# morispi/CONSENT

Measured on AMD Instinct MI355X. Metric: corrected windows/sec, higher is better.
Workload: dtype u8/int16 (2-bit bases, integer DP); 1 GPU; pacbio_d150_msa150: synthetic PacBio-profile piles, 500 bp windows, depth 150, maxMSA 150, k=9, solid=4, commonKMers=8, minAnchors=2; distinct_windows_per_run=704512, engines_per_gpu=4, engines_requested=4, engine_allocation_runs=0, hw_queues=4, overflow_windows=0, template_fallback_windows=0

## Files before the change

consent_amd/csrc/cw_index.h:

```cpp
#ifndef CW_INDEX_H
#define CW_INDEX_H

#include "cw_device.h"

typedef __attribute__((address_space(3))) uint32_t* cw_l32w;
typedef __attribute__((address_space(3))) const uint32_t* cw_l32;
typedef __attribute__((address_space(1))) const uint32_t* cw_g32;
typedef __attribute__((address_space(3))) uint16_t* cw_l16w;
typedef __attribute__((address_space(1))) uint16_t* cw_g16w;
#define CW_IDX_THREADS 1024
#define CW_IDX_WAVES 16
#define CW_IDX_LDS_BYTES 163840
#define CW_TMAX 2048
#define CW_EX_SLOTS 1024
#define CW_EX_BITS 10
#define CW_EXP_SLOTS 8
#define CW_EXG_SLOTS 262144
#define CW_TH_SLOTS 4096
#ifndef CW_IDX_BYTES_MIN_N
#define CW_IDX_BYTES_MIN_N 64u
#endif
#define CW_IDX_STAGE_OFF 139776
#define CW_IDX_STAGE_N 192
#define CW_IDX_STAGE_WORDS ((CW_IDX_LDS_BYTES - CW_IDX_STAGE_OFF - 16 - CW_IDX_STAGE_N * 8) / 4)

enum CwIdxRoute : unsigned {
    CW_IR_STAGED = 1u << 0,
    CW_IR_BYTES_DONE = 1u << 1,
    CW_IR_NIBBLES = 1u << 2,
    CW_IR_BIG_EX = 1u << 3,
    CW_IR_EXPORT_MASKS = 1u << 4,
    CW_IR_EXPORT_WALK = 1u << 5,
    CW_IR_REWALK = 1u << 6,
    CW_IR_HASHED = 1u << 7,
    CW_IR_HASH_PASSES = 1u << 8,
    CW_IR_HASH_GSORT = 1u << 9,
    CW_IR_WIDE = 1u << 10,
    CW_IR_TFIT = 1u << 11,
    CW_IR_PG = 1u << 12,
    CW_IR_HIT_LIST = 1u << 13,
    CW_IR_USE_BITS = 1u << 14
};
#ifdef CW_TEST_AIDS
#define CW_IDX_ROUTE(ctr, cond, bits) do { if (cond) atomicOr(&(ctr)->prof[CW_PS_IDX_ROUTE], (unsigned long long)(bits)); } while (0)
#else
#define CW_IDX_ROUTE(ctr, cond, bits) do { } while (0)
#endif

__host__ __device__ __forceinline__ uint32_t cw_ab_np(uint32_t N) { uint32_t Np = (N + 1u) & ~1u; if (((Np >> 1) & 1u) == 0u) Np += 2u; return Np; }
__host__ __device__ __forceinline__ uint64_t cw_ab_align(uint64_t x) { return (x + 15ull) & ~15ull; }
#define CW_AB_HDR 64u
#define CW_AB_ROWS_MAX 254u
__host__ __device__ __forceinline__ uint32_t cw_ab_ap(uint32_t A) { return (A + 15u) & ~15u; }
template <typename B> struct CwAbCarve {
    B hdr;
    B ckey;
    B pres;
    B dirty;
    B badm;
    B rowid;
    B delta;
    B P;
    B end;
};
template <typename B> __host__ __device__ __forceinline__ CwAbCarve<B> cw_ab_carve(B blk, uint32_t A, uint32_t N, uint32_t n_dirty, uint32_t n_rows) {
    const uint32_t Np = cw_ab_np(N), Nw = (N + 63u) >> 6;
    CwAbCarve<B> c;
    c.hdr = blk;
    c.ckey = blk + CW_AB_HDR;
    c.pres = c.ckey + cw_ab_align((uint64_t)A * 4);
    c.dirty = c.pres + cw_ab_align((uint64_t)A * Nw * 8);
    c.badm = c.dirty + cw_ab_align((uint64_t)n_dirty * 2);
    c.rowid = c.badm + cw_ab_align((uint64_t)A * 8);
    c.delta = c.rowid + cw_ab_align((uint64_t)A);
// ... 105 lines not shown
__device__ __forceinline__ int cw_tpl_lookup(const uint32_t* th, const uint32_t* tkey, uint32_t key) {
    uint32_t bkt = CW_TH_HOME(key);
    const uint32_t fp = CW_TH_FP(key);
    for (;;) {
        for (uint32_t j = 0; j < 4u; ++j) {
            const uint32_t e = th[bkt * 4u + j];
            if (e == 0) return -1;
            if ((e & ~4095u) == fp && tkey[CW_TH_POS(e) - 1] == key) return (int)CW_TH_POS(e) - 1;
        }
        bkt = (bkt + 1) & (CW_TH_BUCKETS - 1);
    }
}

#define CW_IDX_EX_OFF 131072u
#define CW_IDX_SCAN_OFF (CW_IDX_EX_OFF + CW_EX_SLOTS * 8u)
static_assert(CW_IDX_SCAN_OFF + 512u == CW_IDX_STAGE_OFF, "the staged pile starts behind the 512 B of flags and scan scratch");
template <uint32_t T> struct IdxTplOff {
    static constexpr uint32_t tkey = CW_TH_SLOTS * 4u, tsup = tkey + 4u * T, trep = tsup + 4u * T, tcand = trep + T, cand_tp = tcand + 2u * T,
                              seen = cand_tp + 2u * T, misc = seen + CW_IDX_WAVES * (T / 32u) * 4u, P = misc + 256u;
};
static_assert(IdxTplOff<1024>::tsup == 20480u && IdxTplOff<1024>::trep == 24576u && IdxTplOff<1024>::tcand == 25600u && IdxTplOff<1024>::cand_tp == 27648u &&
              IdxTplOff<1024>::seen == 29696u && IdxTplOff<1024>::misc == 31744u && IdxTplOff<1024>::P == 32000u, "the narrow layout");
static_assert(IdxTplOff<2048>::tsup == 24576u && IdxTplOff<2048>::trep == 32768u && IdxTplOff<2048>::tcand == 34816u && IdxTplOff<2048>::cand_tp == 38912u &&
              IdxTplOff<2048>::seen == 43008u && IdxTplOff<2048>::misc == 47104u && IdxTplOff<2048>::P == 47360u, "the wide layout");
static_assert(IdxTplOff<2048>::P < CW_IDX_STAGE_OFF && IdxTplOff<CW_TMAX>::P == IdxTplOff<2048>::P, "the position matrix stops short of the staged pile");

struct IdxLds {
    uint8_t* lds;
    bool wide;
    __device__ __forceinline__ uint32_t* tab() const { return (uint32_t*)lds; }
    __device__ __forceinline__ unsigned long long* ex() const { return (unsigned long long*)(lds + CW_IDX_EX_OFF); }
    __device__ __forceinline__ uint32_t* scan_tmp() const { return (uint32_t*)(lds + CW_IDX_SCAN_OFF); }
    __device__ __forceinline__ uint32_t* flags() const { return scan_tmp() + 32; }
    __device__ __forceinline__ uint32_t* st_hdr() const { return (uint32_t*)(lds + CW_IDX_STAGE_OFF); }
    __device__ __forceinline__ uint32_t* s_len() const { return st_hdr() + 4; }
    __device__ __forceinline__ uint32_t* s_off() const { return s_len() + CW_IDX_STAGE_N; }
    __device__ __forceinline__ uint32_t* s_words() const { return s_off() + CW_IDX_STAGE_N; }
    typedef IdxTplOff<1024> O1; typedef IdxTplOff<2048> O2;
    __device__ __forceinline__ uint32_t* th() const { return (uint32_t*)lds; }
    __device__ __forceinline__ uint32_t* tkey() const { return (uint32_t*)(lds + O1::tkey); }
    __device__ __forceinline__ uint32_t* tsup() const { return (uint32_t*)(lds + (wide ? O2::tsup : O1::tsup)); }
    __device__ __forceinline__ uint8_t* trep() const { return lds + (wide ? O2::trep : O1::trep); }
    __device__ __forceinline__ int16_t* tcand() const { return (int16_t*)(lds + (wide ? O2::tcand : O1::tcand)); }
    __device__ __forceinline__ uint16_t* cand_tp() const { return (uint16_t*)(lds + (wide ? O2::cand_tp : O1::cand_tp)); }
    __device__ __forceinline__ uint32_t* seen() const { return (uint32_t*)(lds + (wide ? O2::seen : O1::seen)); }
    __device__ __forceinline__ uint32_t seen_words() const { return wide ? 64u : 32u; }
    __device__ __forceinline__ uint32_t* misc() const { return (uint32_t*)(lds + (wide ? O2::misc : O1::misc)); }
    __device__ __forceinline__ uint16_t* P() const { return (uint16_t*)(lds + (wide ? O2::P : O1::P)); }
    __device__ __forceinline__ uint32_t p_cap() const { return (CW_IDX_STAGE_OFF - (wide ? O2::P : O1::P)) / 2u; }
};

struct IdxWin {
    WinInfo* wi;
    uint32_t N, L0, solid_base, solid_cap, ab_cap, ab_base, n_kmers;
    __device__ __forceinline__ explicit IdxWin(WinInfo* w) : wi(w), N(w->n_seqs), L0(w->tpl_len), solid_base(w->solid_base), solid_cap(w->solid_cap),
                                                             ab_cap(w->ab_cap), ab_base(w->ab_base), n_kmers(w->n_kmers) {}
};

struct IdxPile {
    uint32_t N, s0;
    bool stm, stw;
    const uint32_t* s_len; const uint32_t* s_off; const uint32_t* s_words;
    const uint32_t* seq_len; const uint64_t* seq_word_off; const uint32_t* bases;
};

struct IdxMatrix {
    uint16_t* P_lds; uint16_t* P_glb;
    const uint16_t* cand_tp;
    bool pg;
    bool tfit;
    uint32_t Np;
    __device__ __forceinline__ uint32_t rd(const uint32_t i) const { return pg ? (uint32_t)((cw_g16w)P_glb)[i] : (uint32_t)((cw_l16w)P_lds)[i]; }
    __device__ __forceinline__ void wr(const uint32_t i, const uint32_t v) const { if (pg) ((cw_g16w)P_glb)[i] = (uint16_t)v; else ((cw_l16w)P_lds)[i] = (uint16_t)v; }
    __device__ __forceinline__ uint32_t row(const uint32_t a) const { return tfit ? (uint32_t)cand_tp[a] : a; }
    __device__ __forceinline__ void clear_lds(const uint32_t n16) const {
        const uint32_t nv = n16 >> 3, pat = (uint32_t)CW_NONE16 * 0x00010001u;
        for (uint32_t i = threadIdx.x; i < nv; i += CW_IDX_THREADS) ((uint4*)P_lds)[i] = make_uint4(pat, pat, pat, pat);
        for (uint32_t i = (nv << 3) + threadIdx.x; i < n16; i += CW_IDX_THREADS) P_lds[i] = (uint16_t)CW_NONE16;
    }
};
__device__ __forceinline__ uint64_t idx_matrix_need(const uint32_t rows, const uint32_t N, const uint32_t Np) {
    return (uint64_t)rows * Np * 2 + (uint64_t)rows * ((N + 63u) >> 6) * 8 + (uint64_t)N * 2 + 16;
}

__device__ __forceinline__ unsigned long long* idx_wg_scratch(const DevScratch& sc) { return sc.ex_fallback + (size_t)blockIdx.x * CW_EXG_SLOTS; }

__device__ __forceinline__ void idx_stop(WinInfo* wi, BatchCounters* ctr, const uint32_t why) { wi->status = CW_WIN_OVERFLOW; wi->pad_ = why; ctr->any_overflow = 1; }

enum IdxShape { IDX_8x128, IDX_8x128_ROT, IDX_2x512, IDX_WAVE };

template <typename W> __device__ __forceinline__ uint64_t idx_window(const W words, const uint32_t p, const uint32_t nwd) {
    const uint32_t wi_ = p >> 4;
    const uint64_t x_ = ((uint64_t)words[wi_] << 32) | (wi_ + 1u < nwd ? words[wi_ + 1u] : 0u);
    return x_ << (2u * (p & 15u));
}
__device__ __forceinline__ uint32_t idx_key_top(const uint64_t x, const uint32_t k) { return (uint32_t)(x >> (64u - 2u * k)); }
__device__ __forceinline__ uint32_t idx_key_field(const uint32_t yh, const uint32_t q, const uint32_t k) { return yh >> (32u - 2u * k - 2u * q); }
__device__ __forceinline__ void idx_keys4(uint64_t x_, const uint32_t k, const uint32_t kmask, uint32_t (&key4)[4]) {
    if (k <= 13u) {
        const uint32_t yh = (uint32_t)(x_ >> 32);
#pragma unroll
        for (uint32_t q = 0; q < 4u; ++q) key4[q] = idx_key_field(yh, q, k) & kmask;
    } else {
// ... 180 lines not shown
}
template <uint32_t KPW, typename Accept, typename CountOf>
__device__ __forceinline__ bool idx_export_masks(const uint32_t (&m)[8], const uint32_t* tab, const uint32_t NI, const uint32_t key_base, const uint32_t out_base,
                                                 uint32_t* scan_tmp, uint32_t* solid_key, uint32_t* solid_cnt, uint32_t& total, Accept&& accept, CountOf&& count_of) {
    const uint32_t lane = threadIdx.x & 63u;
    const uint32_t qbase = (threadIdx.x >> 6) * (NI * 64u) + lane;
    uint32_t offs[8], wtot = 0;
#pragma unroll
    for (int i = 0; i < 8; ++i) {
        const uint32_t c = (uint32_t)__popc(m[i]);
        const uint32_t inc = (uint32_t)cw_wave_scan_add((int)c);
        offs[i] = wtot + inc - c;
        wtot += (uint32_t)cw_lane_value((int)inc, 63);
    }
    uint32_t woff = cw_block_exscan(lane == 0 ? wtot : 0u, scan_tmp, &total);
    woff = (uint32_t)cw_lane_value((int)woff, 0);
    if (!accept(total)) return false;
#pragma unroll
    for (int i = 0; i < 8; ++i) {
        uint32_t mm = m[i], o = out_base + woff + offs[i];
        const uint32_t wd0 = (qbase + (uint32_t)i * 64u) * 4u;
        while (mm) {
            const uint32_t bpos = (uint32_t)__ffs((int)mm) - 1u;
            mm &= mm - 1u;
            const uint32_t wd = wd0 + bpos / KPW, q = bpos & (KPW - 1u), key = key_base + wd * KPW + q;
            solid_key[o] = key;
            solid_cnt[o] = count_of(tab[wd], q, key);
            ++o;
        }
    }
    return true;
}

__device__ __forceinline__ bool idx_count_bytes(const IdxLds& L, const IdxPile& pl, const IdxWin& win, const DevScratch& sc, const cw_params& prm, const uint32_t kmask,
                                                const uint32_t n_keys, bool& done8, unsigned long long& _pt) {
    const int tid = threadIdx.x, lane = tid & 63;
    const uint32_t N = pl.N;
    uint32_t* const tab = L.tab(); uint32_t* const flags = L.flags();
    done8 = false;
    const uint32_t bkeys = n_keys < 131072u ? n_keys : 131072u, bwords = bkeys >> 2, BNI = bwords >> 12;
    if (!(N <= 200u && (n_keys <= 131072u || N >= CW_IDX_BYTES_MIN_N) && prm.solid >= 1u && prm.solid <= 127u && (bwords & 4095u) == 0u && BNI >= 1u && BNI <= 8u)) return true;
    const uint32_t n_half = n_keys / bkeys;
    uint32_t written = 0;
    bool ok8 = true, fits8 = true;
    if (tid < 8) flags[tid] = 0;
    for (uint32_t h = 0; h < n_half; ++h) {
        for (uint32_t i = tid; i < bwords; i += CW_IDX_THREADS) tab[i] = 0;
        __syncthreads();
        if (h == 0) CW_PROF(sc.ctr, CW_PS_IDX_STAGE, tid == 0);
        const uint32_t half_off = h * bkeys;
        idx_pile_pass<IDX_8x128_ROT>(pl, prm.k, kmask, [&](const uint32_t, const uint32_t, const uint32_t key, const uint32_t keyraw) {
            const uint32_t off = (key & ~3u) - half_off;
            if (off >= bkeys) return;
            (void)__hip_atomic_fetch_add((cw_l32w)((__attribute__((address_space(3))) uint8_t*)tab + off), 1u << ((keyraw << 3) & 31u), __ATOMIC_RELAXED, __HIP_MEMORY_SCOPE_WORKGROUP);
        });
        __syncthreads();
        CW_PROF(sc.ctr, CW_PS_IDX_COUNT, tid == 0);
        if (flags[0]) { ok8 = false; break; }
        const uint32_t addt = (128u - prm.solid) * 0x01010101u;
        uint32_t m[8], bsum = 0;
        idx_read_masks<4>(tab, BNI, m, [&](const uint32_t v) -> uint32_t {
            const uint32_t c = (((v & 0x7F7F7F7Fu) + addt) | v) & 0x80808080u;
            bsum = __builtin_amdgcn_sad_u8(v, 0u, bsum);
            return ((c >> 7) | (c >> 14) | (c >> 21) | (c >> 28)) & 0xFu;
        });
        { const uint32_t ws_ = (uint32_t)cw_wave_sum((int)bsum); if (lane == 0) atomicAdd(&flags[2], ws_); }
        CW_PROF(sc.ctr, CW_PS_IDX_EXPORT_SCAN, tid == 0);
        uint32_t total;
        const bool wrote = idx_export_masks<4>(m, tab, BNI, h * 131072u, win.solid_base + written, L.scan_tmp(), sc.solid_key, sc.solid_cnt, total,
            [&](const uint32_t n) -> bool {
                if (h + 1u == n_half && flags[2] != win.n_kmers) { ok8 = false; return false; }
                fits8 = written + n <= win.solid_cap;
                if (!fits8 && h + 1u != n_half) ok8 = false;
                return fits8;
            },
            [&](const uint32_t v, const uint32_t q, const uint32_t) -> uint32_t { return (v >> (8u * q)) & 255u; });
        if (!wrote) break;
        written += total;
        __syncthreads();
    }
    if (ok8) {
        if (tid == 0) {
            win.wi->n_solid = fits8 ? written : 0;
            if (!fits8) idx_stop(win.wi, sc.ctr, CW_WHY_SOLIDCAP);
        }
        __syncthreads();
        if (!fits8) return false;
        done8 = true;
    }
// ... 202 lines not shown
    const int tid = threadIdx.x;
    const unsigned long long* const exg = idx_wg_scratch(sc);
    uint32_t total;
    bool fits;
    const uint32_t NI = nib_words >> 12;
    if (prm.solid <= 15u && (nib_words & 4095u) == 0u && NI >= 1u && NI <= 8u) {
        const uint32_t add = (16u - (prm.solid < 15u ? prm.solid : 15u)) * 0x01010101u;
        uint32_t m[8];
        CW_IDX_ROUTE(sc.ctr, tid == 0, CW_IR_EXPORT_MASKS);
        idx_read_masks<8>(L.tab(), NI, m, [&](const uint32_t v) -> uint32_t {
            const uint32_t c = idx_nibble_cand(v, add);
            return (c | (c >> 6) | (c >> 12) | (c >> 18)) & 0xFFu;
        });
        CW_PROF(sc.ctr, CW_PS_IDX_EXPORT_SCAN, tid == 0);
        fits = idx_export_masks<8>(m, L.tab(), NI, 0u, win.solid_base, L.scan_tmp(), sc.solid_key, sc.solid_cnt, total,
            [&](const uint32_t n) -> bool { return n <= win.solid_cap; },
            [&](const uint32_t v, const uint32_t q, const uint32_t key) -> uint32_t {
                uint32_t c = (v >> (4u * q)) & 15u;
                if (c == 15u) c += idx_ex_lookup(L.ex(), exg, big_ex, key);
                return c;
            });
    } else {
        CW_IDX_ROUTE(sc.ctr, tid == 0, CW_IR_EXPORT_WALK);
        fits = idx_export_walk(L, win, sc, prm, n_keys, nib_words, exg, big_ex, total, _pt);
    }
    if (tid == 0) {
        win.wi->n_solid = fits ? total : 0;
        if (!fits) idx_stop(win.wi, sc.ctr, CW_WHY_SOLIDCAP);
    }
    __syncthreads();
    return fits;
}

__device__ __forceinline__ void idx_template_table(const IdxLds& L, const IdxPile& pl, const IdxMatrix& M, const uint32_t k, const uint32_t nk0) {
    const int tid = threadIdx.x;
    uint32_t* const th = L.th(); uint32_t* const tkey = L.tkey();
    if (M.tfit) M.clear_lds(nk0 * M.Np);
    if (tid == 0) { L.misc()[4] = 0; L.misc()[5] = 0; }
    for (uint32_t i = tid; i < CW_TH_SLOTS; i += CW_IDX_THREADS) th[i] = 0;
    for (uint32_t i = tid; i < L.seen_words() * 32u; i += CW_IDX_THREADS) { L.tsup()[i] = 0; L.trep()[i] = 0; L.tcand()[i] = -1; }
    for (uint32_t tp = tid; tp < nk0; tp += CW_IDX_THREADS) tkey[tp] = pl.stw ? cw_kmer_at(pl.s_words, tp, k) : cw_kmer_at(pl.bases + pl.seq_word_off[pl.s0], tp, k);
    __syncthreads();
    for (uint32_t tp = tid; tp < nk0; tp += CW_IDX_THREADS) {
        const uint32_t key = tkey[tp];
        uint32_t bkt = CW_TH_HOME(key);
        for (bool placed = false; !placed; bkt = (bkt + 1) & (CW_TH_BUCKETS - 1)) {
            for (uint32_t j = 0; j < 4u && !placed; ++j) {
                const uint32_t prev = atomicCAS(&th[bkt * 4u + j], 0u, (tp + 1u) | CW_TH_FP(key));
                if (prev == 0) placed = true;
                else if ((prev & ~4095u) == CW_TH_FP(key) && tkey[CW_TH_POS(prev) - 1] == key) { L.trep()[CW_TH_POS(prev) - 1] = 1; placed = true; }
            }
        }
    }
    __syncthreads();
}

#define CW_IDX_HIT_CAP (CW_EXG_SLOTS * 2u)
__device__ __forceinline__ bool idx_hit_list(const IdxMatrix& M, const uint32_t N) { return !M.tfit && N <= 1024u; }

__device__ __forceinline__ void idx_support(const IdxLds& L, const IdxPile& pl, const IdxMatrix& M, const DevScratch& sc, const uint32_t k, const uint32_t kmask) {
    const int lane = threadIdx.x & 63, wave = threadIdx.x >> 6;
    const uint32_t N = pl.N, Np = M.Np;
    uint32_t* const th = L.th(); uint32_t* const tkey = L.tkey(); uint32_t* const tsup = L.tsup(); uint8_t* const trep = L.trep(); uint32_t* const misc = L.misc();
    uint16_t* const P_lds = M.P_lds;
    const bool tfit = M.tfit, hl = idx_hit_list(M, N);
    uint32_t* const hitlist = (uint32_t*)idx_wg_scratch(sc);
    const uint32_t hit_cap = CW_IDX_HIT_CAP;
    const bool fp_exact = k <= 10u;
    auto support_seq = [&](const auto words, const uint32_t len, const uint32_t s, uint32_t* my_seen) {
        const uint32_t nk = len >= k ? len - k + 1 : 0, nwd = (len + 15u) >> 4;
        for (uint32_t p0 = (uint32_t)lane * 4u; p0 < nk; p0 += 256u) {
            uint32_t key4[4], bkt4[4], e1[4];
            idx_keys4(idx_window(words, p0, nwd), k, kmask, key4);
#pragma unroll
            for (uint32_t q = 0; q < 4u; ++q) bkt4[q] = CW_TH_HOME(key4[q]);
            if (fp_exact) {
                auto match = [&](const uint4 v, const uint32_t fp1) -> uint32_t { return min(min(v.x - fp1, v.y - fp1), min(v.z - fp1, v.w - fp1)); };
                uint4 v4[4];
#pragma unroll
                for (uint32_t q = 0; q < 4u; ++q) v4[q] = p0 + q < nk ? *(const uint4*)&th[bkt4[q] * 4u] : make_uint4(0u, 0u, 0u, 0u);
                uint32_t pend = 0;
#pragma unroll
                for (uint32_t q = 0; q < 4u; ++q) { e1[q] = match(v4[q], CW_TH_FP(key4[q]) + 1u); if (e1[q] >= (uint32_t)CW_TMAX && v4[q].w != 0u) pend |= 1u << q; }
                while (__ballot(pend != 0u) != 0ull) {
#pragma unroll
                    for (uint32_t q = 0; q < 4u; ++q) {
                        if ((pend >> q) & 1u) {
                            bkt4[q] = (bkt4[q] + 1u) & (CW_TH_BUCKETS - 1);
                            const uint4 v = *(const uint4*)&th[bkt4[q] * 4u];
                            e1[q] = match(v, CW_TH_FP(key4[q]) + 1u);
                            if (e1[q] < (uint32_t)CW_TMAX || v.w == 0u) pend &= ~(1u << q);
                        }
                    }
                }
            } else {
#pragma unroll
                for (uint32_t q = 0; q < 4u; ++q) e1[q] = p0 + q < nk ? (uint32_t)cw_tpl_lookup(th, tkey, key4[q]) : 0xFFFFFFFFu;
            }
            uint32_t old4[4];
#pragma unroll
            for (uint32_t q = 0; q < 4u; ++q) {
                const uint32_t e = e1[q];
                old4[q] = e < (uint32_t)CW_TMAX ? atomicOr(&my_seen[e >> 5], 1u << (e & 31u)) : 0u;
            }
            uint32_t n_list = 0, my_list = 0;
#pragma unroll
            for (uint32_t q = 0; q < 4u; ++q) {
                const uint32_t e = e1[q], p = p0 + q;
                const bool hit = e < (uint32_t)CW_TMAX;
                if (hit) {
                    if (old4[q] & (1u << (e & 31u))) trep[e] = 1;
                    else atomicAdd(&tsup[e], 1u);
                    if (tfit) P_lds[__umul24(e, Np) + s] = (uint16_t)p;
                    else if (hl && p >= 2048u) misc[5] = 1;
                }
                if (!tfit && hl) {
                    const unsigned long long hm = __ballot(hit && p < 2048u);
                    if (hit && p < 2048u) my_list |= (n_list + (uint32_t)__popcll(hm & ((1ull << lane) - 1ull))) << (8u * q);
                    n_list += (uint32_t)__popcll(hm);
                }
            }
            if (!tfit && hl && n_list) {
                uint32_t base = 0;
                if (lane == 0) base = atomicAdd(&misc[4], n_list);
                base = (uint32_t)cw_lane_value((int)base, 0);
#pragma unroll
                for (uint32_t q = 0; q < 4u; ++q) {
                    const uint32_t p = p0 + q, hi_ = base + ((my_list >> (8u * q)) & 255u);
                    if (e1[q] < (uint32_t)CW_TMAX && p < 2048u && hi_ < hit_cap) hitlist[hi_] = (e1[q] << 21) | (s << 11) | p;
                }
            }
        }
    };
    for (uint32_t s = wave; s < N; s += CW_IDX_WAVES) {
        uint32_t* my_seen = L.seen() + wave * L.seen_words();
        if ((uint32_t)lane < L.seen_words()) my_seen[lane] = 0;
        cw_wave_sync();
        idx_with_seq(pl, s, [&](const auto words, const uint32_t len) { support_seq(words, len, s, my_seen); });
        cw_wave_sync();
    }
    __syncthreads();
}

__device__ __forceinline__ uint32_t idx_candidates(const IdxLds& L, const uint32_t nk0, const int sup_min) {
    const int tid = threadIdx.x;
    uint32_t A = 0;
    for (uint32_t tb = 0; tb < nk0; tb += CW_IDX_THREADS) {
        const uint32_t tp = tb + (uint32_t)tid;
        uint32_t ok = 0;
        if (tp < nk0) {
            const int rep = cw_tpl_lookup(L.th(), L.tkey(), L.tkey()[tp]);
            ok = (rep == (int)tp && L.trep()[tp] == 0 && (int)L.tsup()[tp] >= sup_min) ? 1u : 0u;
        }
        uint32_t a_round;
        const uint32_t off = A + cw_block_exscan(ok, L.scan_tmp(), &a_round);
        if (ok) { L.tcand()[tp] = (int16_t)off; L.cand_tp()[off] = (uint16_t)tp; }
        A += a_round;
        __syncthreads();
    }
    __syncthreads();
    return A;
}

__device__ __forceinline__ bool idx_fill_matrix(const IdxLds& L, const IdxPile& pl, const IdxWin& win, const IdxMatrix& M, const DevScratch& sc, const uint32_t k, const uint32_t kmask,
                                                const uint32_t A) {
    const int tid = threadIdx.x, wave = tid >> 6;
    const uint32_t N = pl.N, Np = M.Np;
    if (M.pg && (uint64_t)A * Np > sc.p_fallback_elems) {
        if (tid == 0) { idx_stop(win.wi, sc.ctr, CW_WHY_MATRIX); win.wi->arena_used = (uint64_t)A * Np > 0xFFFFFFFFull ? 0xFFFFFFFFu : A * Np; }
        __builtin_amdgcn_wave_barrier();
        return false;
    }
    const uint32_t* const hitlist = (const uint32_t*)idx_wg_scratch(sc);
    const uint32_t n_hits = L.misc()[4];
    const bool from_list = idx_hit_list(M, N) && n_hits <= CW_IDX_HIT_CAP && L.misc()[5] == 0u;
    if (!M.tfit) {
        if (!M.pg) M.clear_lds(A * Np);
        else for (uint32_t i = tid; i < A * Np; i += CW_IDX_THREADS) M.wr(i, CW_NONE16);
        __builtin_amdgcn_fence(__ATOMIC_RELEASE, "workgroup");
        __syncthreads();
        __builtin_amdgcn_fence(__ATOMIC_ACQUIRE, "workgroup");
        if (from_list) {
            for (uint32_t i0 = tid; i0 < n_hits; i0 += 4u * CW_IDX_THREADS) {
                uint32_t h4[4];
#pragma unroll
                for (uint32_t u = 0; u < 4u; ++u) { const uint32_t i = i0 + u * CW_IDX_THREADS; h4[u] = i < n_hits ? hitlist[i] : 0xFFFFFFFFu; }
#pragma unroll
                for (uint32_t u = 0; u < 4u; ++u) {
                    const uint32_t h = h4[u];
                    const int a = i0 + u * CW_IDX_THREADS < n_hits ? L.tcand()[h >> 21] : -1;
                    if (a >= 0) M.wr((uint32_t)a * Np + ((h >> 11) & 1023u), h & 2047u);
                }
            }
        } else
        for (uint32_t s = wave; s < N; s += CW_IDX_WAVES) {
            idx_pile_seq<IDX_WAVE>(pl, s, k, kmask, [&](const uint32_t, const uint32_t p, const uint32_t key, const uint32_t) {
                const int e = cw_tpl_lookup(L.th(), L.tkey(), key);
                if (e < 0) return;
                const int a = L.tcand()[e];
                if (a >= 0) M.wr((uint32_t)a * Np + s, p);
            });
        }
        __syncthreads();
    }
    return true;
}

struct IdxPres {
    uint8_t* clean;
    uint8_t* didx;
    unsigned long long* pres;
    uint16_t* dirty;
    unsigned long long* badm;
    uint8_t* rowid;
    uint16_t* rowanc;
    bool use_bits, has_bm, has_delta;
    uint32_t n_rows;
    uint32_t W;
    uint32_t n_dirty;
};
__device__ __forceinline__ IdxPres idx_presence_carve(const IdxLds& L, const IdxMatrix& M, const uint32_t A, const uint32_t N, const uint32_t nk0) {
    uint8_t* const lds = L.lds;
    const uint32_t Nw = (N + 63u) >> 6;
    IdxPres ps;
// ... 152 lines not shown
    {
        const uint32_t* src = (const uint32_t*)(M.pg ? M.P_glb : M.P_lds);
        uint32_t* dst = (uint32_t*)ab.P;
        const uint32_t half = Np >> 1;
        if (M.tfit) {
            for (uint32_t a = wave; a < A; a += CW_IDX_WAVES)
                for (uint32_t j = lane; j < half; j += 64) dst[a * half + j] = src[(uint32_t)L.cand_tp()[a] * half + j];
        } else {
            const uint32_t n2 = A * half;
            if (!M.pg) {
                const uint32_t n4 = n2 >> 2;
                for (uint32_t i = tid; i < n4; i += CW_IDX_THREADS) ((uint4*)dst)[i] = ((const uint4*)src)[i];
                for (uint32_t i = (n4 << 2) + tid; i < n2; i += CW_IDX_THREADS) dst[i] = src[i];
            } else
            for (uint32_t i = tid; i < n2; i += CW_IDX_THREADS) dst[i] = src[i];
        }
    }
    return true;
}

__global__ void __launch_bounds__(CW_IDX_THREADS) cw_index_kernel(DevBatch b, DevScratch sc, cw_params prm) {
    extern __shared__ __attribute__((aligned(16))) uint8_t lds[];
    const int tid = threadIdx.x;
    const uint32_t k = prm.k;
    const bool direct = k <= 9;
    const uint32_t n_keys = direct ? 1u << (2 * k) : 0u;
    const uint32_t kmask = k >= 16u ? 0xFFFFFFFFu : (1u << (2u * k)) - 1u;
    const uint32_t nib_words = direct ? (n_keys >= 8 ? n_keys / 8 : 1) : 0u;
    IdxLds L;
    L.lds = lds; L.wide = false;

    for (;;) {
        __syncthreads();
        if (tid == 0) { L.st_hdr()[1] = atomicAdd(&sc.ctr->next_window, 1u); L.st_hdr()[0] = 0; }
        __syncthreads();
        const uint32_t w = L.st_hdr()[1];
        if (w >= b.n_windows) break;
        WinInfo* wi = &sc.win[w];
        if (wi->status == CW_WIN_OVERFLOW) continue;
        const uint32_t s0 = b.win_first_seq[w];
        const IdxWin win(wi);
        const uint32_t N = win.N, L0 = win.L0;
        L.wide = L0 >= k && L0 - k + 1u > 1024u;
        const IdxPile pl = idx_stage_pile(b, L, s0, N);
        CW_IDX_ROUTE(sc.ctr, tid == 0, (pl.stw ? CW_IR_STAGED : 0u) | (L.wide ? CW_IR_WIDE : 0u));
        CW_PROF_T0();
        if (!direct) {
            if (!idx_count_hashed(L, pl, win, sc, prm, kmask)) continue;
        } else {
            bool done8, big_ex;
            if (!idx_count_bytes(L, pl, win, sc, prm, kmask, n_keys, done8, _pt)) continue;
            CW_IDX_ROUTE(sc.ctr, tid == 0, done8 ? CW_IR_BYTES_DONE : CW_IR_NIBBLES);
            if (!done8) {
                if (!idx_count_nibbles(L, pl, win, sc, prm, kmask, nib_words, big_ex, _pt)) continue;
                CW_IDX_ROUTE(sc.ctr, tid == 0 && big_ex, CW_IR_BIG_EX);
                if (!idx_export_nibbles(L, win, sc, prm, n_keys, nib_words, big_ex, _pt)) continue;
            }
        }
        CW_PROF(sc.ctr, CW_PS_IDX_EXPORT, tid == 0);
        const uint32_t nk0 = L0 >= k ? L0 - k + 1 : 0;
        const int sup_min = min((int)prm.common_kmers, (int)N / 2);
        if (nk0 == 0 || nk0 > CW_TMAX) {
            if (tid == 0) {
                if (nk0 == 0) wi->status = CW_WIN_TEMPLATE;
                else idx_stop(wi, sc.ctr, CW_WHY_TEMPLATE);
            }
            __builtin_amdgcn_wave_barrier();
            continue;
        }
        IdxMatrix M;
        M.P_lds = L.P(); M.P_glb = sc.p_fallback + (size_t)blockIdx.x * sc.p_fallback_elems; M.cand_tp = L.cand_tp();
        M.Np = cw_ab_np(N);
        M.pg = false;
        M.tfit = idx_matrix_need(nk0, N, M.Np) <= (uint64_t)L.p_cap() * 2;
        idx_template_table(L, pl, M, k, nk0);
        CW_PROF(sc.ctr, CW_PS_IDX_TPLHASH, tid == 0);
        idx_support(L, pl, M, sc, k, kmask);
        CW_PROF(sc.ctr, CW_PS_IDX_SUPPORT, tid == 0);
        const uint32_t A = idx_candidates(L, nk0, sup_min);
        CW_PROF(sc.ctr, CW_PS_IDX_CAND, tid == 0);
        M.pg = !M.tfit && idx_matrix_need(A, N, M.Np) > (uint64_t)L.p_cap() * 2;
        CW_IDX_ROUTE(sc.ctr, tid == 0, (M.tfit ? CW_IR_TFIT : 0u) | (M.pg ? CW_IR_PG : 0u) | (idx_hit_list(M, N) ? CW_IR_HIT_LIST : 0u));
        if (!idx_fill_matrix(L, pl, win, M, sc, k, kmask, A)) continue;
        CW_PROF(sc.ctr, CW_PS_IDX_PFILL, tid == 0);
        IdxPres ps = idx_presence_carve(L, M, A, N, nk0);
        CW_IDX_ROUTE(sc.ctr, tid == 0 && ps.use_bits, CW_IR_USE_BITS);
        if (ps.use_bits) {
            ps = idx_classify_sequences(L, win, M, ps, sc, A, _pt);
            CW_PROF(sc.ctr, CW_PS_IDX_DIRTY, tid == 0);
            idx_presence(M, ps, A, N);
            ps.n_dirty = L.misc()[3];
        }
        CW_PROF(sc.ctr, CW_PS_IDX_PRESENCE, tid == 0);
        if (!idx_hand_over(L, win, M, ps, sc, A)) continue;
        CW_PROF(sc.ctr, CW_PS_IDX_HANDOVER, tid == 0);
    }
}

#endif
```

consent_amd/engine.py:

```python
import ctypes as C
import os

import numpy as np

WIN_CONSENSUS, WIN_TEMPLATE, WIN_OVERFLOW = 0, 1, 2
SW_ALIGNED, SW_NO_INDELS, SW_STOP, SW_IS_REF = 0, 1, 2, 3
SW_SCORE, SW_REF_BEGIN, SW_REF_END, SW_QUERY_BEGIN, SW_QUERY_END, SW_INS, SW_DEL, SW_STATUS, SW_ROW = 0, 1, 2, 3, 4, 5, 6, 7, 8
SW_WANT_INDELS = 1
SW_QMAX, SW_RMAX, SW_DIR_BYTES = 32768, 16383, 1 << 20
SW_NO_PATH, SW_PATH_OPEN, SW_PATH_SLOT = 4, 5, 6
SW_PATH_EQX = 4
SW_OP_M, SW_OP_I, SW_OP_D, SW_OP_EQ, SW_OP_X = 0, 1, 2, 7, 8
SW_PATH_BYTES = 2 << 20
SW_OP_LETTERS = {SW_OP_M: "M", SW_OP_I: "I", SW_OP_D: "D", SW_OP_EQ: "=", SW_OP_X: "X"}
SW_PILE_SLOT = 7
PILE_ACCUMULATE = 8
PILE_A, PILE_C, PILE_G, PILE_T, PILE_DEL, PILE_INS, PILE_BEGIN, PILE_END, PILE_COL = 0, 1, 2, 3, 4, 5, 6, 7, 8
SW_CUT_SLOT = 8
STRAND_FWD, STRAND_REV, STRAND_IS_REF, STRAND_NONE = 0, 1, 2, 3
STRAND_K, STRAND_KMIN, STRAND_KMAX = 11, 8, 15
SEED_STATUS, SEED_HITS, SEED_DIAG, SEED_OTHER, SEED_ROW = 0, 1, 2, 3, 4
SEED_SHIFT = 6
SEED_SPAN = 2 << SEED_SHIFT
SEED_MIN_HITS, SEED_MIN_K = 14, 11
# ... 195 lines not shown
                                            C.c_void_p, C.c_void_p, C.c_void_p, C.c_void_p, C.c_uint32, C.c_uint64, C.POINTER(C.c_uint32), C.POINTER(C.c_uint64), C.c_void_p]
    lib.cw_stitch_device.argtypes = [C.c_void_p, C.POINTER(ReadSet), C.c_void_p, C.c_uint32, C.c_void_p, C.POINTER(Batch), C.POINTER(Result), C.c_uint32, C.c_uint32,
                                     C.c_int32, C.c_void_p, C.c_void_p, C.c_void_p, C.c_void_p, C.c_void_p]
    lib.cw_index_reads.argtypes = [C.c_char_p, C.POINTER(C.c_void_p)]
    lib.cw_index_reads_append.argtypes = [C.c_void_p, C.c_char_p]
    lib.cw_read_index_free.argtypes = [C.c_void_p]
    lib.cw_read_index_free.restype = None
    lib.cw_read_index_count.argtypes = [C.c_void_p]
    lib.cw_read_index_count.restype = C.c_uint32
    lib.cw_read_index_view.argtypes = [C.c_void_p, C.POINTER(ReadSet), C.POINTER(C.c_uint64)]
    lib.cw_read_index_find.argtypes = [C.c_void_p, C.c_char_p]
    lib.cw_read_index_find.restype = C.c_int32
    lib.cw_read_index_name.argtypes = [C.c_void_p, C.c_uint32]
    lib.cw_read_index_name.restype = C.c_char_p
    lib.cw_paf_open.argtypes = [C.c_char_p, C.c_void_p, C.c_uint32, C.POINTER(C.c_void_p)]
    lib.cw_paf_next_pile.argtypes = [C.c_void_p, C.POINTER(C.c_uint32), C.POINTER(C.c_uint32), C.c_void_p, C.c_void_p, C.c_uint32, C.POINTER(C.c_uint32)]
    lib.cw_paf_close.argtypes = [C.c_void_p]
    lib.cw_paf_close.restype = None
    lib.cw_paf_reformat.argtypes = [C.c_char_p, C.c_char_p]
    lib.cw_paf_explode.argtypes = [C.c_char_p, C.c_char_p, C.POINTER(C.c_uint32)]
    lib.cw_paf_merge.argtypes = [C.c_char_p, C.c_char_p, C.POINTER(C.c_char_p), C.c_uint32]
    lib.cw_window_positions.argtypes = [C.c_uint32, C.c_void_p, C.c_uint32, C.c_uint32, C.c_uint32, C.c_int32, C.c_void_p, C.c_uint32, C.POINTER(C.c_uint32)]
    lib.cw_pack_sequence.argtypes = [C.c_char_p, C.c_uint32, C.c_void_p, C.c_uint64]
    lib.cw_pack_sequence.restype = C.c_int64
    lib.cw_synth_sizes.argtypes = [C.POINTER(SynthSpec), C.POINTER(C.c_uint32), C.POINTER(C.c_uint64)]
    lib.cw_synth_host.argtypes = [C.POINTER(SynthSpec), C.c_void_p, C.c_void_p, C.c_void_p, C.c_void_p]
    lib.cw_synth_device.argtypes = [C.c_void_p, C.POINTER(SynthSpec), C.c_void_p, C.c_void_p, C.c_void_p, C.c_void_p, C.c_void_p]
    _LIBS[p] = lib
    return lib


INDEX_ROUTE_SLOT = 63
INDEX_ROUTE = {"staged": 1 << 0, "bytes_done": 1 << 1, "nibbles": 1 << 2, "big_ex": 1 << 3, "export_masks": 1 << 4, "export_walk": 1 << 5, "rewalk": 1 << 6,
               "hashed": 1 << 7, "hash_passes": 1 << 8, "hash_gsort": 1 << 9, "wide": 1 << 10, "tfit": 1 << 11, "pg": 1 << 12, "hit_list": 1 << 13, "use_bits": 1 << 14}


CHAIN_ROUTE_SLOT = 45
CHAIN_ROUTE = {"fast": 1 << 0, "rows_lds": 1 << 1, "rows_far": 1 << 2, "pres_lds": 1 << 3, "wide_key": 1 << 4, "far_scan": 1 << 5, "inplace_rows": 1 << 6,
               "inplace_masks": 1 << 7, "inplace_all_dirty": 1 << 8, "inplace_matrix": 1 << 9, "early_flush": 1 << 10, "long_single": 1 << 11, "long_slab": 1 << 12}


FINISH_ROUTE_SLOT = 33
FINISH_ROUTE = {"staged": 1 << 0, "compact": 1 << 1, "global": 1 << 2, "cnt16": 1 << 3, "cnt_global": 1 << 4, "vis_lds": 1 << 5, "vis_global": 1 << 6, "find4": 1 << 7,
                "count_scan": 1 << 8, "head": 1 << 9, "tail": 1 << 10, "linked": 1 << 11, "first_pass": 1 << 12, "second_pass": 1 << 13}


def route_names(bits, table=None):
    return sorted(n for n, b in (table or INDEX_ROUTE).items() if bits & b)


def _check(lib, rc, what, allow_capacity=False):
    if rc == 0 or (allow_capacity and rc == -4):
        return rc
    raise EngineError(f"{what}: {lib.cw_strerror(rc).decode()} ({rc})")


def _ptr(a):
    return C.c_void_p(a.ctypes.data)


class HostBatch:

    def __init__(self, win_first_seq, seq_len, seq_word_off, bases):
        self.win_first_seq = np.ascontiguousarray(win_first_seq, np.uint32)
        self.seq_len = np.ascontiguousarray(seq_len, np.uint32)
        self.seq_word_off = np.ascontiguousarray(seq_word_off, np.uint64)
        self.bases = np.ascontiguousarray(bases, np.uint32)
# ... 850 lines not shown
```

Baseline: 302,600 windows/s.

## Prefilter template k-mers by byte-count support before building template table

While the byte count table is still live, each template k-mer position is checked against the minimum support threshold and the result is stored as a ballot bitmask in the extra LDS region. The template key list is then compacted to only eligible k-mers with a block exclusive scan, so the template hash, support, candidate and matrix stages work on fewer positions. This can also let the position matrix fit in LDS more often. The cost is an extra pass over template k-mers per count half, plus a scan with block syncs per 1024 positions.

```diff
diff --git a/consent_amd/csrc/cw_index.h b/consent_amd/csrc/cw_index.h
--- a/consent_amd/csrc/cw_index.h
+++ b/consent_amd/csrc/cw_index.h
@@ -39,7 +39,8 @@
     CW_IR_TFIT = 1u << 11,
     CW_IR_PG = 1u << 12,
     CW_IR_HIT_LIST = 1u << 13,
-    CW_IR_USE_BITS = 1u << 14
+    CW_IR_USE_BITS = 1u << 14,
+    CW_IR_ELIG = 1u << 15
 };
 #ifdef CW_TEST_AIDS
 #define CW_IDX_ROUTE(ctr, cond, bits) do { if (cond) atomicOr(&(ctr)->prof[CW_PS_IDX_ROUTE], (unsigned long long)(bits)); } while (0)
@@ -211,6 +212,7 @@
     __device__ __forceinline__ unsigned long long* ex() const { return (unsigned long long*)(lds + CW_IDX_EX_OFF); }
     __device__ __forceinline__ uint32_t* scan_tmp() const { return (uint32_t*)(lds + CW_IDX_SCAN_OFF); }
     __device__ __forceinline__ uint32_t* flags() const { return scan_tmp() + 32; }
+    __device__ __forceinline__ unsigned long long* elig() const { return ex(); }
     __device__ __forceinline__ uint32_t* st_hdr() const { return (uint32_t*)(lds + CW_IDX_STAGE_OFF); }
     __device__ __forceinline__ uint32_t* s_len() const { return st_hdr() + 4; }
     __device__ __forceinline__ uint32_t* s_off() const { return s_len() + CW_IDX_STAGE_N; }
@@ -494,6 +496,12 @@
     return true;
 }
 
+__device__ __forceinline__ int idx_sup_min(const cw_params& prm, const uint32_t N) { return min((int)prm.common_kmers, (int)N / 2); }
+
+__device__ __forceinline__ uint32_t idx_template_kmer(const IdxPile& pl, const uint32_t tp, const uint32_t k) {
+    return pl.stw ? cw_kmer_at(pl.s_words, tp, k) : cw_kmer_at(pl.bases + pl.seq_word_off[pl.s0], tp, k);
+}
+
 __device__ __forceinline__ bool idx_count_bytes(const IdxLds& L, const IdxPile& pl, const IdxWin& win, const DevScratch& sc, const cw_params& prm, const uint32_t kmask,
                                                 const uint32_t n_keys, bool& done8, unsigned long long& _pt) {
     const int tid = threadIdx.x, lane = tid & 63;
@@ -517,6 +525,19 @@
             (void)__hip_atomic_fetch_add((cw_l32w)((__attribute__((address_space(3))) uint8_t*)tab + off), 1u << ((keyraw << 3) & 31u), __ATOMIC_RELAXED, __HIP_MEMORY_SCOPE_WORKGROUP);
         });
         __syncthreads();
+        const uint32_t nkt = win.L0 >= prm.k && win.L0 - prm.k < (uint32_t)CW_TMAX ? win.L0 - prm.k + 1u : 0u;
+        const int sup_min = idx_sup_min(prm, N);
+#pragma nounroll
+        for (uint32_t tb = 0; tb < nkt; tb += CW_IDX_THREADS) {
+            const uint32_t tp = tb + (uint32_t)tid;
+            bool el = false;
+            if (tp < nkt) {
+                const uint32_t off = idx_template_kmer(pl, tp, prm.k) - half_off;
+                if (off < bkeys) el = (int)((const uint8_t*)tab)[off] >= sup_min;
+            }
+            const unsigned long long bal = __ballot(el);
+            if (lane == 0) L.elig()[tp >> 6] = h ? L.elig()[tp >> 6] | bal : bal;
+        }
         CW_PROF(sc.ctr, CW_PS_IDX_COUNT, tid == 0);
         if (flags[0]) { ok8 = false; break; }
         const uint32_t addt = (128u - prm.solid) * 0x01010101u;
@@ -785,14 +806,35 @@
     return fits;
 }
 
-__device__ __forceinline__ void idx_template_table(const IdxLds& L, const IdxPile& pl, const IdxMatrix& M, const uint32_t k, const uint32_t nk0) {
+__device__ __forceinline__ uint32_t idx_template_keys(const IdxLds& L, const IdxPile& pl, const uint32_t k, const uint32_t nk0, const bool elig) {
+    const int tid = threadIdx.x;
+    uint32_t* const tkey = L.tkey();
+    if (!elig) {
+        for (uint32_t tp = tid; tp < nk0; tp += CW_IDX_THREADS) tkey[tp] = idx_template_kmer(pl, tp, k);
+        return nk0;
+    }
+    uint32_t E = 0;
+#pragma nounroll
+    for (uint32_t tb = 0; tb < nk0; tb += CW_IDX_THREADS) {
+        const uint32_t tp = tb + (uint32_t)tid;
+        const uint32_t el = tp < nk0 ? (uint32_t)(L.elig()[tp >> 6] >> (tp & 63u)) & 1u : 0u;
+        const uint32_t key = el ? idx_template_kmer(pl, tp, k) : 0u;
+        uint32_t e_round;
+        const uint32_t d = E + cw_block_exscan(el, L.scan_tmp(), &e_round);
+        if (el) tkey[d] = key;
+        E += e_round;
+        __syncthreads();
+    }
+    return E;
+}
+
+__device__ __forceinline__ void idx_template_table(const IdxLds& L, const IdxMatrix& M, const uint32_t nk0) {
     const int tid = threadIdx.x;
     uint32_t* const th = L.th(); uint32_t* const tkey = L.tkey();
     if (M.tfit) M.clear_lds(nk0 * M.Np);
     if (tid == 0) { L.misc()[4] = 0; L.misc()[5] = 0; }
     for (uint32_t i = tid; i < CW_TH_SLOTS; i += CW_IDX_THREADS) th[i] = 0;
     for (uint32_t i = tid; i < L.seen_words() * 32u; i += CW_IDX_THREADS) { L.tsup()[i] = 0; L.trep()[i] = 0; L.tcand()[i] = -1; }
-    for (uint32_t tp = tid; tp < nk0; tp += CW_IDX_THREADS) tkey[tp] = pl.stw ? cw_kmer_at(pl.s_words, tp, k) : cw_kmer_at(pl.bases + pl.seq_word_off[pl.s0], tp, k);
     __syncthreads();
     for (uint32_t tp = tid; tp < nk0; tp += CW_IDX_THREADS) {
         const uint32_t key = tkey[tp];
@@ -1174,10 +1216,11 @@
         const IdxPile pl = idx_stage_pile(b, L, s0, N);
         CW_IDX_ROUTE(sc.ctr, tid == 0, (pl.stw ? CW_IR_STAGED : 0u) | (L.wide ? CW_IR_WIDE : 0u));
         CW_PROF_T0();
+        bool done8 = false;
         if (!direct) {
             if (!idx_count_hashed(L, pl, win, sc, prm, kmask)) continue;
         } else {
-            bool done8, big_ex;
+            bool big_ex;
             if (!idx_count_bytes(L, pl, win, sc, prm, kmask, n_keys, done8, _pt)) continue;
             CW_IDX_ROUTE(sc.ctr, tid == 0, done8 ? CW_IR_BYTES_DONE : CW_IR_NIBBLES);
             if (!done8) {
@@ -1188,7 +1231,7 @@
         }
         CW_PROF(sc.ctr, CW_PS_IDX_EXPORT, tid == 0);
         const uint32_t nk0 = L0 >= k ? L0 - k + 1 : 0;
-        const int sup_min = min((int)prm.common_kmers, (int)N / 2);
+        const int sup_min = idx_sup_min(prm, N);
         if (nk0 == 0 || nk0 > CW_TMAX) {
             if (tid == 0) {
                 if (nk0 == 0) wi->status = CW_WIN_TEMPLATE;
@@ -1201,18 +1244,20 @@
         M.P_lds = L.P(); M.P_glb = sc.p_fallback + (size_t)blockIdx.x * sc.p_fallback_elems; M.cand_tp = L.cand_tp();
         M.Np = cw_ab_np(N);
         M.pg = false;
-        M.tfit = idx_matrix_need(nk0, N, M.Np) <= (uint64_t)L.p_cap() * 2;
-        idx_template_table(L, pl, M, k, nk0);
+        const uint32_t E = idx_template_keys(L, pl, k, nk0, done8);
+        CW_IDX_ROUTE(sc.ctr, tid == 0 && done8 && E < nk0, CW_IR_ELIG);
+        M.tfit = idx_matrix_need(E, N, M.Np) <= (uint64_t)L.p_cap() * 2;
+        idx_template_table(L, M, E);
         CW_PROF(sc.ctr, CW_PS_IDX_TPLHASH, tid == 0);
         idx_support(L, pl, M, sc, k, kmask);
         CW_PROF(sc.ctr, CW_PS_IDX_SUPPORT, tid == 0);
-        const uint32_t A = idx_candidates(L, nk0, sup_min);
+        const uint32_t A = idx_candidates(L, E, sup_min);
         CW_PROF(sc.ctr, CW_PS_IDX_CAND, tid == 0);
         M.pg = !M.tfit && idx_matrix_need(A, N, M.Np) > (uint64_t)L.p_cap() * 2;
         CW_IDX_ROUTE(sc.ctr, tid == 0, (M.tfit ? CW_IR_TFIT : 0u) | (M.pg ? CW_IR_PG : 0u) | (idx_hit_list(M, N) ? CW_IR_HIT_LIST : 0u));
         if (!idx_fill_matrix(L, pl, win, M, sc, k, kmask, A)) continue;
         CW_PROF(sc.ctr, CW_PS_IDX_PFILL, tid == 0);
-        IdxPres ps = idx_presence_carve(L, M, A, N, nk0);
+        IdxPres ps = idx_presence_carve(L, M, A, N, E);
         CW_IDX_ROUTE(sc.ctr, tid == 0 && ps.use_bits, CW_IR_USE_BITS);
         if (ps.use_bits) {
             ps = idx_classify_sequences(L, win, M, ps, sc, A, _pt);
diff --git a/consent_amd/engine.py b/consent_amd/engine.py
--- a/consent_amd/engine.py
+++ b/consent_amd/engine.py
@@ -251,7 +251,8 @@
 
 INDEX_ROUTE_SLOT = 63
 INDEX_ROUTE = {"staged": 1 << 0, "bytes_done": 1 << 1, "nibbles": 1 << 2, "big_ex": 1 << 3, "export_masks": 1 << 4, "export_walk": 1 << 5, "rewalk": 1 << 6,
-               "hashed": 1 << 7, "hash_passes": 1 << 8, "hash_gsort": 1 << 9, "wide": 1 << 10, "tfit": 1 << 11, "pg": 1 << 12, "hit_list": 1 << 13, "use_bits": 1 << 14}
+               "hashed": 1 << 7, "hash_passes": 1 << 8, "hash_gsort": 1 << 9, "wide": 1 << 10, "tfit": 1 << 11, "pg": 1 << 12, "hit_list": 1 << 13, "use_bits": 1 << 14,
+               "elig": 1 << 15}
 
 
 CHAIN_ROUTE_SLOT = 45
```

New measurement: 303,600 windows/s (median of 4 runs). No clear change (+0.3%).

## Replace compacted hit list with per-sequence positional hit map in index fill

Applied to the files above, without the earlier changes.

Support pass now writes, for every k-mer position of each read, a 16-bit template-entry id (or none) into a per-read row of a global scratch map, instead of compacting hits through an LDS atomic counter and ballot/popcount into a packed hit list. Matrix fill then streams each read's map row and scatters the positions whose template entry became a candidate. This removes the per-group atomic, ballot bookkeeping and the 2048-position/capacity fallback, but writes every position (including misses) to global memory and adds a layout check that falls back when sequence offsets overlap or exceed the scratch capacity.

```diff
diff --git a/consent_amd/csrc/cw_index.h b/consent_amd/csrc/cw_index.h
--- a/consent_amd/csrc/cw_index.h
+++ b/consent_amd/csrc/cw_index.h
@@ -39,7 +39,8 @@
     CW_IR_TFIT = 1u << 11,
     CW_IR_PG = 1u << 12,
     CW_IR_HIT_LIST = 1u << 13,
-    CW_IR_USE_BITS = 1u << 14
+    CW_IR_USE_BITS = 1u << 14,
+    CW_IR_HIT_MAP = 1u << 15
 };
 #ifdef CW_TEST_AIDS
 #define CW_IDX_ROUTE(ctr, cond, bits) do { if (cond) atomicOr(&(ctr)->prof[CW_PS_IDX_ROUTE], (unsigned long long)(bits)); } while (0)
@@ -248,6 +249,7 @@
     const uint16_t* cand_tp;
     bool pg;
     bool tfit;
+    bool map;
     uint32_t Np;
     __device__ __forceinline__ uint32_t rd(const uint32_t i) const { return pg ? (uint32_t)((cw_g16w)P_glb)[i] : (uint32_t)((cw_l16w)P_lds)[i]; }
     __device__ __forceinline__ void wr(const uint32_t i, const uint32_t v) const { if (pg) ((cw_g16w)P_glb)[i] = (uint16_t)v; else ((cw_l16w)P_lds)[i] = (uint16_t)v; }
@@ -789,7 +791,6 @@
     const int tid = threadIdx.x;
     uint32_t* const th = L.th(); uint32_t* const tkey = L.tkey();
     if (M.tfit) M.clear_lds(nk0 * M.Np);
-    if (tid == 0) { L.misc()[4] = 0; L.misc()[5] = 0; }
     for (uint32_t i = tid; i < CW_TH_SLOTS; i += CW_IDX_THREADS) th[i] = 0;
     for (uint32_t i = tid; i < L.seen_words() * 32u; i += CW_IDX_THREADS) { L.tsup()[i] = 0; L.trep()[i] = 0; L.tcand()[i] = -1; }
     for (uint32_t tp = tid; tp < nk0; tp += CW_IDX_THREADS) tkey[tp] = pl.stw ? cw_kmer_at(pl.s_words, tp, k) : cw_kmer_at(pl.bases + pl.seq_word_off[pl.s0], tp, k);
@@ -808,19 +809,37 @@
     __syncthreads();
 }
 
-#define CW_IDX_HIT_CAP (CW_EXG_SLOTS * 2u)
+#define CW_IDX_MAP_WORDS CW_EXG_SLOTS
+typedef __attribute__((address_space(1))) unsigned long long* cw_g64w;
 __device__ __forceinline__ bool idx_hit_list(const IdxMatrix& M, const uint32_t N) { return !M.tfit && N <= 1024u; }
+__device__ __forceinline__ uint32_t idx_seq_rel(const IdxPile& pl, const uint32_t s) { return pl.stm ? pl.s_off[s] : (uint32_t)(pl.seq_word_off[pl.s0 + s] - pl.seq_word_off[pl.s0]); }
+__device__ __forceinline__ cw_g64w idx_map_row(const IdxPile& pl, const DevScratch& sc, const uint32_t s) { return (cw_g64w)idx_wg_scratch(sc) + 4u * idx_seq_rel(pl, s); }
+__device__ __forceinline__ void idx_map_check(const IdxLds& L, const IdxPile& pl, const IdxMatrix& M) {
+    if (!idx_hit_list(M, pl.N)) return;
+    const uint32_t cap = CW_IDX_MAP_WORDS / 4u;
+    for (uint32_t s = threadIdx.x; s < pl.N; s += CW_IDX_THREADS) {
+        bool bad;
+        if (pl.stm) {
+            const uint32_t rel = pl.s_off[s], prev_end = s ? pl.s_off[s - 1] + ((pl.s_len[s - 1] + 15u) >> 4) : 0u;
+            bad = rel < prev_end || rel + ((pl.s_len[s] + 15u) >> 4) > cap || L.st_hdr()[0] == 0xFFFFFFFFu;
+        } else {
+            const uint64_t base = pl.seq_word_off[pl.s0], rel = pl.seq_word_off[pl.s0 + s] - base;
+            const uint64_t prev_end = s ? pl.seq_word_off[pl.s0 + s - 1] - base + ((pl.seq_len[pl.s0 + s - 1] + 15u) >> 4) : 0ull;
+            bad = rel < prev_end || rel + ((pl.seq_len[pl.s0 + s] + 15u) >> 4) > cap;
+        }
+        if (bad) L.st_hdr()[2] = 1u;
+    }
+}
+__device__ __forceinline__ bool idx_map_ok(const IdxLds& L, const IdxMatrix& M, const uint32_t N) { return idx_hit_list(M, N) && L.st_hdr()[2] == 0u; }
 
 __device__ __forceinline__ void idx_support(const IdxLds& L, const IdxPile& pl, const IdxMatrix& M, const DevScratch& sc, const uint32_t k, const uint32_t kmask) {
     const int lane = threadIdx.x & 63, wave = threadIdx.x >> 6;
     const uint32_t N = pl.N, Np = M.Np;
-    uint32_t* const th = L.th(); uint32_t* const tkey = L.tkey(); uint32_t* const tsup = L.tsup(); uint8_t* const trep = L.trep(); uint32_t* const misc = L.misc();
+    uint32_t* const th = L.th(); uint32_t* const tkey = L.tkey(); uint32_t* const tsup = L.tsup(); uint8_t* const trep = L.trep();
     uint16_t* const P_lds = M.P_lds;
-    const bool tfit = M.tfit, hl = idx_hit_list(M, N);
-    uint32_t* const hitlist = (uint32_t*)idx_wg_scratch(sc);
-    const uint32_t hit_cap = CW_IDX_HIT_CAP;
+    const bool tfit = M.tfit, map = M.map;
     const bool fp_exact = k <= 10u;
-    auto support_seq = [&](const auto words, const uint32_t len, const uint32_t s, uint32_t* my_seen) {
+    auto support_seq = [&](const auto words, const uint32_t len, const uint32_t s, uint32_t* my_seen, const cw_g64w my_map) {
         const uint32_t nk = len >= k ? len - k + 1 : 0, nwd = (len + 15u) >> 4;
         for (uint32_t p0 = (uint32_t)lane * 4u; p0 < nk; p0 += 256u) {
             uint32_t key4[4], bkt4[4], e1[4];
@@ -856,40 +875,27 @@
                 const uint32_t e = e1[q];
                 old4[q] = e < (uint32_t)CW_TMAX ? atomicOr(&my_seen[e >> 5], 1u << (e & 31u)) : 0u;
             }
-            uint32_t n_list = 0, my_list = 0;
+            uint32_t m4[4];
 #pragma unroll
             for (uint32_t q = 0; q < 4u; ++q) {
-                const uint32_t e = e1[q], p = p0 + q;
+                const uint32_t e = e1[q];
                 const bool hit = e < (uint32_t)CW_TMAX;
+                m4[q] = hit ? e : CW_NONE16;
                 if (hit) {
                     if (old4[q] & (1u << (e & 31u))) trep[e] = 1;
                     else atomicAdd(&tsup[e], 1u);
-                    if (tfit) P_lds[__umul24(e, Np) + s] = (uint16_t)p;
-                    else if (hl && p >= 2048u) misc[5] = 1;
+                    if (tfit) P_lds[__umul24(e, Np) + s] = (uint16_t)(p0 + q);
                 }
-                if (!tfit && hl) {
-                    const unsigned long long hm = __ballot(hit && p < 2048u);
-                    if (hit && p < 2048u) my_list |= (n_list + (uint32_t)__popcll(hm & ((1ull << lane) - 1ull))) << (8u * q);
-                    n_list += (uint32_t)__popcll(hm);
-                }
-            }
-            if (!tfit && hl && n_list) {
-                uint32_t base = 0;
-                if (lane == 0) base = atomicAdd(&misc[4], n_list);
-                base = (uint32_t)cw_lane_value((int)base, 0);
-#pragma unroll
-                for (uint32_t q = 0; q < 4u; ++q) {
-                    const uint32_t p = p0 + q, hi_ = base + ((my_list >> (8u * q)) & 255u);
-                    if (e1[q] < (uint32_t)CW_TMAX && p < 2048u && hi_ < hit_cap) hitlist[hi_] = (e1[q] << 21) | (s << 11) | p;
-                }
-            }
+            }
+            if (map) my_map[p0 >> 2] = (unsigned long long)(m4[0] | (m4[1] << 16)) | ((unsigned long long)(m4[2] | (m4[3] << 16)) << 32);
         }
     };
     for (uint32_t s = wave; s < N; s += CW_IDX_WAVES) {
         uint32_t* my_seen = L.seen() + wave * L.seen_words();
         if ((uint32_t)lane < L.seen_words()) my_seen[lane] = 0;
         cw_wave_sync();
-        idx_with_seq(pl, s, [&](const auto words, const uint32_t len) { support_seq(words, len, s, my_seen); });
+        const cw_g64w my_map = map ? idx_map_row(pl, sc, s) : (cw_g64w)0;
+        idx_with_seq(pl, s, [&](const auto words, const uint32_t len) { support_seq(words, len, s, my_seen, my_map); });
         cw_wave_sync();
     }
     __syncthreads();
@@ -924,25 +930,42 @@
         __builtin_amdgcn_wave_barrier();
         return false;
     }
-    const uint32_t* const hitlist = (const uint32_t*)idx_wg_scratch(sc);
-    const uint32_t n_hits = L.misc()[4];
-    const bool from_list = idx_hit_list(M, N) && n_hits <= CW_IDX_HIT_CAP && L.misc()[5] == 0u;
+    const int lane = tid & 63;
     if (!M.tfit) {
         if (!M.pg) M.clear_lds(A * Np);
         else for (uint32_t i = tid; i < A * Np; i += CW_IDX_THREADS) M.wr(i, CW_NONE16);
         __builtin_amdgcn_fence(__ATOMIC_RELEASE, "workgroup");
         __syncthreads();
         __builtin_amdgcn_fence(__ATOMIC_ACQUIRE, "workgroup");
-        if (from_list) {
-            for (uint32_t i0 = tid; i0 < n_hits; i0 += 4u * CW_IDX_THREADS) {
-                uint32_t h4[4];
-#pragma unroll
-                for (uint32_t u = 0; u < 4u; ++u) { const uint32_t i = i0 + u * CW_IDX_THREADS; h4[u] = i < n_hits ? hitlist[i] : 0xFFFFFFFFu; }
-#pragma unroll
-                for (uint32_t u = 0; u < 4u; ++u) {
-                    const uint32_t h = h4[u];
-                    const int a = i0 + u * CW_IDX_THREADS < n_hits ? L.tcand()[h >> 21] : -1;
-                    if (a >= 0) M.wr((uint32_t)a * Np + ((h >> 11) & 1023u), h & 2047u);
+        if (M.map) {
+            const uint32_t tmask = L.seen_words() * 32u - 1u;
+            const int16_t* const tcand = L.tcand();
+            auto scatter = [&](const unsigned long long w, const uint32_t s, const uint32_t g) {
+                int a4[4];
+#pragma unroll
+                for (uint32_t q = 0; q < 4u; ++q) a4[q] = tcand[(uint32_t)(w >> (16u * q)) & tmask];
+#pragma unroll
+                for (uint32_t q = 0; q < 4u; ++q)
+                    if (((uint32_t)(w >> (16u * q)) & 0xFFFFu) != CW_NONE16 && a4[q] >= 0) M.wr((uint32_t)a4[q] * Np + s, g * 4u + q);
+            };
+            for (uint32_t s0 = wave; s0 < N; s0 += 2u * CW_IDX_WAVES) {
+                uint32_t ng2[2];
+#pragma unroll
+                for (uint32_t u = 0; u < 2u; ++u) {
+                    const uint32_t s = s0 + u * CW_IDX_WAVES;
+                    ng2[u] = 0;
+                    if (s < N) { const uint32_t len = pl.stm ? pl.s_len[s] : pl.seq_len[pl.s0 + s]; ng2[u] = len >= k ? (len - k + 4u) >> 2 : 0u; }
+                }
+                for (uint32_t g0 = (uint32_t)lane; g0 < max(ng2[0], ng2[1]); g0 += 128u) {
+                    unsigned long long w4[2][2];
+#pragma unroll
+                    for (uint32_t u = 0; u < 2u; ++u)
+#pragma unroll
+                        for (uint32_t v = 0; v < 2u; ++v) { const uint32_t g = g0 + v * 64u; w4[u][v] = g < ng2[u] ? idx_map_row(pl, sc, s0 + u * CW_IDX_WAVES)[g] : ~0ull; }
+#pragma unroll
+                    for (uint32_t u = 0; u < 2u; ++u)
+#pragma unroll
+                        for (uint32_t v = 0; v < 2u; ++v) scatter(w4[u][v], s0 + u * CW_IDX_WAVES, g0 + v * 64u);
                 }
             }
         } else
@@ -1161,7 +1184,7 @@
 
     for (;;) {
         __syncthreads();
-        if (tid == 0) { L.st_hdr()[1] = atomicAdd(&sc.ctr->next_window, 1u); L.st_hdr()[0] = 0; }
+        if (tid == 0) { L.st_hdr()[1] = atomicAdd(&sc.ctr->next_window, 1u); L.st_hdr()[0] = 0; L.st_hdr()[2] = 0; }
         __syncthreads();
         const uint32_t w = L.st_hdr()[1];
         if (w >= b.n_windows) break;
@@ -1202,14 +1225,16 @@
         M.Np = cw_ab_np(N);
         M.pg = false;
         M.tfit = idx_matrix_need(nk0, N, M.Np) <= (uint64_t)L.p_cap() * 2;
+        idx_map_check(L, pl, M);
         idx_template_table(L, pl, M, k, nk0);
+        M.map = idx_map_ok(L, M, N);
         CW_PROF(sc.ctr, CW_PS_IDX_TPLHASH, tid == 0);
         idx_support(L, pl, M, sc, k, kmask);
         CW_PROF(sc.ctr, CW_PS_IDX_SUPPORT, tid == 0);
         const uint32_t A = idx_candidates(L, nk0, sup_min);
         CW_PROF(sc.ctr, CW_PS_IDX_CAND, tid == 0);
         M.pg = !M.tfit && idx_matrix_need(A, N, M.Np) > (uint64_t)L.p_cap() * 2;
-        CW_IDX_ROUTE(sc.ctr, tid == 0, (M.tfit ? CW_IR_TFIT : 0u) | (M.pg ? CW_IR_PG : 0u) | (idx_hit_list(M, N) ? CW_IR_HIT_LIST : 0u));
+        CW_IDX_ROUTE(sc.ctr, tid == 0, (M.tfit ? CW_IR_TFIT : 0u) | (M.pg ? CW_IR_PG : 0u) | (idx_hit_list(M, N) ? CW_IR_HIT_LIST : 0u) | (M.map ? CW_IR_HIT_MAP : 0u));
         if (!idx_fill_matrix(L, pl, win, M, sc, k, kmask, A)) continue;
         CW_PROF(sc.ctr, CW_PS_IDX_PFILL, tid == 0);
         IdxPres ps = idx_presence_carve(L, M, A, N, nk0);
diff --git a/consent_amd/engine.py b/consent_amd/engine.py
--- a/consent_amd/engine.py
+++ b/consent_amd/engine.py
@@ -251,7 +251,8 @@
 
 INDEX_ROUTE_SLOT = 63
 INDEX_ROUTE = {"staged": 1 << 0, "bytes_done": 1 << 1, "nibbles": 1 << 2, "big_ex": 1 << 3, "export_masks": 1 << 4, "export_walk": 1 << 5, "rewalk": 1 << 6,
-               "hashed": 1 << 7, "hash_passes": 1 << 8, "hash_gsort": 1 << 9, "wide": 1 << 10, "tfit": 1 << 11, "pg": 1 << 12, "hit_list": 1 << 13, "use_bits": 1 << 14}
+               "hashed": 1 << 7, "hash_passes": 1 << 8, "hash_gsort": 1 << 9, "wide": 1 << 10, "tfit": 1 << 11, "pg": 1 << 12, "hit_list": 1 << 13, "use_bits": 1 << 14,
+               "hit_map": 1 << 15}
 
 
 CHAIN_ROUTE_SLOT = 45
```

After: 302,600 windows/s before, 303,100 windows/s after, median of 2. Within noise of the previous version (+0.2%).
